# HarryShomer/LPFormer

Hardware: AMD Instinct MI355X
Metric: candidate link-pairs scored/sec (whole node) (higher is better)
Workload: dtype f32

## Files before the change

include/lpformer_hip.h:

```cpp
#ifndef LPFORMER_HIP_H
#define LPFORMER_HIP_H

#include <stdint.h>

#ifdef __cplusplus
extern "C" {
#endif

#define LPF_OK 0
#define LPF_ERR_INVALID (-1)
#define LPF_ERR_UNSUPPORTED (-2)
#define LPF_ERR_LAUNCH (-3)
#define LPF_ERR_NO_DEVICE (-4)

#define LPF_ABI_VERSION 10

#define LPF_FLAG_RELU 1u

int lpf_abi_version(void);
const char *lpf_strerror(int code);
const char *lpf_last_hip_error(void);
int lpf_device_info(int *cu_count, int *lds_bytes_per_cu, int *wave_size, char *arch_name, int arch_name_len);


int lpf_gcn_norm_csr(int64_t n, const int64_t *rowptr, const int32_t *col, const float *w_in,
                     float *w_out, float *dis_tmp, void *stream);

#define LPF_SPMM_LONG_ROW 128
int lpf_spmm_csr_f32(int64_t n, int32_t D, const int64_t *rowptr, const int32_t *col, const float *w,
                     const float *H, int64_t ldh, float *out, int64_t ldo, const float *bias,
// ... 215 lines not shown
                                 const float *pe_tab_signed, const float *pe_stat, const float *pat_base,
                                 const void *pat_grid, const void *pat_sign, int32_t grid_n, int32_t grid_shift,
                                 int32_t grid_base, float grid_ofs, const float *wfold_t, const float *att, const float *att_bias,
                                 const float *ln_g, const float *ln_b, int32_t n_counts, const int64_t *sel_ctl,
                                 float *pieces, int64_t units_cap, float *out, int64_t ldo, int32_t *perm,
                                 int64_t *n_nonempty, void *stream);
int lpf_pair_attention_rows4_zbf16(int32_t D, int64_t bs, const void *pair_tab, const int32_t *blk_cnt,
                                   const void *entries, int64_t ent_cap, const void *Z_bf16, int64_t ldz, const float *q,
                                   int64_t ldq, const float *pe_tab_signed, const float *pe_stat, const float *pat_base,
                                   const void *pat_grid, const void *pat_sign, int32_t grid_n, int32_t grid_shift,
                                   int32_t grid_base, float grid_ofs, const float *wfold_t, const float *att, const float *att_bias,
                                   const float *ln_g, const float *ln_b, int32_t n_counts, const int64_t *sel_ctl,
                                   float *pieces, int64_t units_cap, float *out, int64_t ldo, int32_t *perm,
                                   int64_t *n_nonempty, void *stream);

int lpf_tail_chain_rows_perm_f32(int64_t M, int32_t D, int32_t n_counts, const float *rows, int64_t ldrows,
                                 const float *wB_packed, const float *bB, const float *lnB_g, const float *lnB_b,
                                 const float *r_e, int64_t ldre, const float *wC_packed, const float *bC,
                                 const float *w_dot, const float *b_dot, const int64_t *sel_ctl, const int32_t *perm,
                                 const int64_t *n_full, const float *bC_empty, const float *row_empty, float *logit,
                                 float *prob, void *stream);
int lpf_tail_chain_rows_perm_bf16(int64_t M, int32_t D, int32_t n_counts, const float *rows, int64_t ldrows,
                                  const void *wB_packed_bf16, const float *bB, const float *lnB_g, const float *lnB_b,
                                  const float *r_e, int64_t ldre, const void *wC_packed_bf16, const float *bC,
                                  const float *w_dot, const float *b_dot, const int64_t *sel_ctl, const int32_t *perm,
                                  const int64_t *n_full, const float *bC_empty, const float *row_empty, float *logit,
                                  float *prob, void *stream);

int lpf_rowdot_sigmoid_f32(int64_t M, int32_t K, const float *A, int64_t lda, const float *w, float b,
                           float *logit, float *prob, void *stream);
// ... 64 lines not shown
```

lpformer_amd/_lib.py:

```python
from __future__ import annotations

import ctypes as C
import os
import threading

_HERE = os.path.dirname(os.path.abspath(__file__))
HIP_LIB_PATH = os.path.join(_HERE, "liblpformer_hip.so")
HOST_LIB_PATH = os.path.join(_HERE, "liblpformer_host.so")

ABI_VERSION = 10
FLAG_RELU = 1
SELECT_ERR_NODE_RANGE, SELECT_ERR_ITEM_CAP, SELECT_ERR_ENTRY_CAP = 1, 2, 4
ROWS_PERM_LB_WORDS = 1025
SELECT4_BLOCK = 64

i32, i64, f32, f64, u32, u64, vp = C.c_int32, C.c_int64, C.c_float, C.c_double, C.c_uint32, C.c_uint64, C.c_void_p

HIP_PROTOTYPES = {
    "lpf_abi_version": [],
    "lpf_strerror": [C.c_int],
    "lpf_last_hip_error": [],
    "lpf_device_info": [C.POINTER(C.c_int), C.POINTER(C.c_int), C.POINTER(C.c_int), C.c_char_p, C.c_int],
    "lpf_gcn_norm_csr": [i64, vp, vp, vp, vp, vp, vp],
    "lpf_spmm_csr_f32": [i64, i32, vp, vp, vp, vp, i64, vp, i64, vp, vp, vp, vp, i64, vp, vp, u32, vp, i64, vp],
    "lpf_gemm_f32": [i64, i32, i32, vp, i64, vp, i64, vp, vp, i64, vp, i64, u32, vp],
# ... 32 lines not shown
    "lpf_pair_attention_flip_f32": [i32, i64, vp, vp, i64, vp, i64, vp, i64, vp, vp, vp, vp, vp, vp, vp, i64, vp],
    "lpf_pair_attention_flip_zbf16": [i32, i64, vp, vp, i64, vp, i64, vp, i64, vp, vp, vp, vp, vp, vp, vp, i64, vp],
    "lpf_pair_attention_merge_f32": [i64, i32, i32, vp, vp, i64, vp, vp, vp, vp, vp, vp, i64, vp],
    "lpf_pair_attention_rows_f32": [i32, i64, vp, vp, i64, vp, i64, vp, i64, vp, vp, vp, vp, vp, vp, vp, vp, i32, vp, vp,
                                    i64, vp, i64, vp],
    "lpf_pair_attention_rows_zbf16": [i32, i64, vp, vp, i64, vp, i64, vp, i64, vp, vp, vp, vp, vp, vp, vp, vp, i32, vp, vp,
                                      i64, vp, i64, vp],
    "lpf_pair_attention_rows_perm_f32": [i32, i64, vp, vp, i64, vp, i64, vp, i64, vp, vp, vp, vp, vp, vp, vp, vp, i32, vp,
                                         vp, i64, vp, i64, vp, vp, vp, vp],
    "lpf_pair_attention_rows_perm_zbf16": [i32, i64, vp, vp, i64, vp, i64, vp, i64, vp, vp, vp, vp, vp, vp, vp, vp, i32,
                                           vp, vp, i64, vp, i64, vp, vp, vp, vp],
    "lpf_pair_attention_rows4_f32": [i32, i64, vp, vp, vp, i64, vp, i64, vp, i64, vp, vp, vp, vp, vp, i32, i32, i32, f32, vp,
                                     vp, vp, vp, vp, i32, vp, vp, i64, vp, i64, vp, vp, vp],
    "lpf_pair_attention_rows4_zbf16": [i32, i64, vp, vp, vp, i64, vp, i64, vp, i64, vp, vp, vp, vp, vp, i32, i32, i32, f32, vp,
                                       vp, vp, vp, vp, i32, vp, vp, i64, vp, i64, vp, vp, vp],
    "lpf_tail_chain_rows_perm_f32": [i64, i32, i32, vp, i64, vp, vp, vp, vp, vp, i64, vp, vp, vp, vp, vp, vp, vp, vp, vp,
                                     vp, vp, vp],
    "lpf_tail_chain_rows_perm_bf16": [i64, i32, i32, vp, i64, vp, vp, vp, vp, vp, i64, vp, vp, vp, vp, vp, vp, vp, vp, vp,
                                      vp, vp, vp],
    "lpf_pair_rows_piece_floats": [i32],
    "lpf_tail_chain_rows_f32": [i64, i32, i32, vp, i64, vp, vp, vp, vp, vp, i64, vp, vp, vp, vp, vp, vp, vp, vp],
    "lpf_tail_chain_rows_bf16": [i64, i32, i32, vp, i64, vp, vp, vp, vp, vp, i64, vp, vp, vp, vp, vp, vp, vp, vp],
    "lpf_tail_chain_merge_f32": [i64, i32, i32, vp, vp, i64, vp, vp, vp, vp, vp, vp, vp, vp, vp, i64, vp, vp, vp, vp, vp,
                                 vp, vp, vp],
    "lpf_tail_chain_merge_bf16": [i64, i32, i32, vp, vp, i64, vp, vp, vp, vp, vp, vp, vp, vp, vp, i64, vp, vp, vp, vp, vp,
                                 vp, vp, vp],
    "lpf_rowdot_sigmoid_f32": [i64, i32, vp, i64, vp, f32, vp, vp, vp],
    "lpf_tail_chain_f32": [i64, i32, i32, vp, i64, vp, vp, vp, vp, i64, vp, vp, vp, vp, vp, i64, vp, vp, vp, vp, vp,
                           vp, vp],
    "lpf_ppr_filter_count": [i64, vp, vp, i32, f32, vp, vp],
# ... 139 lines not shown
```

lpformer_amd/csrc/pair_rows.hip:

```cpp
#include <type_traits>

#include "pe_common.h"
#include "select_common.h"

namespace {

constexpr uint32_t PR_PAIR_MASK = 0x7fffffffu;
constexpr int PR_LB_WORDS = LPF_ROWS_PERM_LB_WORDS - 1;
#ifndef PR_CHUNK_N
#define PR_CHUNK_N 512
#endif
#ifndef PR_FLAGS_N
#define PR_FLAGS_N 2048
#endif
constexpr int PR_CHUNK = PR_CHUNK_N;
constexpr int PR_FLAGS = PR_FLAGS_N;

struct RowsArgs {
    int64_t bs;
    const int32_t *type_ptr;
    const int4 *entries;
    int64_t ent_cap;
    const float *Z; uint32_t ldz;
    const float *q; uint32_t ldq;
// ... 6 lines not shown
    float *out; int64_t ldo;
    int32_t n_counts;
    const int64_t *sel_ctl;
    float *pieces;
    int64_t units_cap;
    int32_t *perm;
    uint64_t *perm_lb;
    int64_t *n_nonempty;
    const int4 *pair_tab;
    const int32_t *blk_cnt;
    const float *pat_base;
    const uint8_t *pat_grid;
    const uint32_t *pat_sign;
    int32_t grid_n, grid_shift, grid_base;
    float grid_ofs;
};

template <int CTRL>
__device__ __forceinline__ float pr_dpp(float v) {
    return __builtin_bit_cast(float, __builtin_amdgcn_update_dpp(0, __builtin_bit_cast(int, v), CTRL, 0xf, 0xf, false));
}
template <int G>
__device__ __forceinline__ float pr_group_sum(float v) {
    v += pr_dpp<0xB1>(v);
    v += pr_dpp<0x4E>(v);
    if constexpr (G >= 8) v += pr_dpp<0x141>(v);
    if constexpr (G >= 16) v += pr_dpp<0x140>(v);
    if constexpr (G >= 32)
        v += __builtin_bit_cast(float, __builtin_amdgcn_ds_swizzle(__builtin_bit_cast(int, v), 0x401f));
    if constexpr (G >= 64) {
// ... 32 lines not shown
    static constexpr int WT = STAT + 6;
    static constexpr int REC = WT + (PT ? 0 : WTL) * D * GG;
    static constexpr int SC = REC + NG * 16;
    static constexpr int META = SC + NG * 8;
    static constexpr int TP = META + NG * 4;
    static constexpr int CUM = TP + 3 * (PR_CHUNK / 4 + 1);
    static constexpr int LISTS = CUM + (PR_CHUNK / 4 + 1);
    static constexpr int CTL = LISTS + 2 * (PR_CHUNK / 4);
    static constexpr int FLAGS = CTL + 4;
    static constexpr int WCNT = FLAGS + PR_FLAGS / 4;
    static constexpr int SIGN = WCNT + 8;
    static constexpr int TOTAL = SIGN + (PT ? (3 * NP * ((D + 31) / 32) + 3) / 4 : 0);
    static constexpr size_t BYTES = (size_t)TOTAL * 16;
};

template <int G, int NTH, int WTL_, bool ZB = false, bool PT = false, int NV = 1>
__global__ __launch_bounds__(NTH, NTH >= 512 ? 4 : 3) void pair_rows_kernel(const RowsArgs A) {
    using ZT = typename std::conditional<ZB, uint2, float4>::type;
    using L = PrLds<G, NTH, WTL_, PT, NV>;
    constexpr int WTL = PT ? 0 : WTL_, NP = L::NP, GG = L::GG;
    constexpr int D = 4 * GG, EPW = 64 / G, NG = L::NG, T_LO = WTL == 1 ? 1 : 0, TPS = PR_CHUNK + 4, RSP = pr_piece_floats(D);
    constexpr uint32_t PAIR_MASK = PT ? 0x1fffffffu : PR_PAIR_MASK;
    constexpr int SB = LPF_SELECT4_BLOCK;
    constexpr int EW = 4;
    extern __shared__ __attribute__((aligned(16))) float4 pr_lds[];
    float4 *const ltab = pr_lds + L::TAB;
    float4 *const lbase = pr_lds + L::BASE;
    float4 *const lvec = pr_lds + L::VEC;
    float4 *const lconst = pr_lds + L::CONST_ROW;
    float *const lstat = reinterpret_cast<float *>(pr_lds + L::STAT);
    float4 *const lwt = pr_lds + L::WT;
    int4 *const lrec = reinterpret_cast<int4 *>(pr_lds + L::REC);
    f32x2 *const lsc = reinterpret_cast<f32x2 *>(pr_lds + L::SC);
    int *const lmeta = reinterpret_cast<int *>(pr_lds + L::META);
    int *const ltp = reinterpret_cast<int *>(pr_lds + L::TP);
    int *const lcum = reinterpret_cast<int *>(pr_lds + L::CUM);
    int *const llist = reinterpret_cast<int *>(pr_lds + L::LISTS);
    int *const lctl = reinterpret_cast<int *>(pr_lds + L::CTL);
// ... 361 lines not shown
        if constexpr (ZB)
            return make_float4(__uint_as_float(z.x << 16), __uint_as_float(z.x & 0xffff0000u),
                               __uint_as_float(z.y << 16), __uint_as_float(z.y & 0xffff0000u));
        else
            return z;
    };
    auto grid_cell = [&](float v) __attribute__((always_inline)) {
        const int c = (int)(__float_as_uint(v + A.grid_ofs) >> A.grid_shift) - A.grid_base;
        return c < 0 ? A.grid_n - 1 : (c < A.grid_n ? c : A.grid_n - 1);
    };
    auto q_row = [&](int pair, float4 (&q)[NV]) __attribute__((always_inline)) {
#pragma unroll
        for (int v = 0; v < NV; ++v)
            q[v] = *reinterpret_cast<const float4 *>(A.q + (uint64_t)(uint32_t)pair * A.ldq + off + 4 * G * v);
    };

    for (int64_t c0 = P0; c0 < P1; c0 += PR_CHUNK) {
        const int cn = (int)(P1 - c0 < PR_CHUNK ? P1 - c0 : PR_CHUNK);
        constexpr int PER = (PR_CHUNK + NTH - 1) / NTH;
        int4 e_pre[PER];
        if constexpr (PT) {
#pragma unroll
            for (int i = 0; i < PER; ++i) {
                const int k = tid * PER + i;
                e_pre[i] = A.pair_tab[c0 + (k < cn ? k : cn - 1)];
            }
        }
        pr_lds_barrier();
        int64_t v0, v1;
        if constexpr (PT) {
// ... 55 lines not shown
        const int64_t u_first = v0 >> 4;
        const int n_units = v1 > v0 ? (int)(((v1 - 1) >> 4) - u_first + 1) : 0;
        const bool inl = n_units <= PR_FLAGS;
        if (inl)
            for (int k = tid; k < n_units; k += NTH) lflag[k] = 0;
        pr_lds_barrier();
        PR_STAMP(2);
        PR_STAMP(3);
        while (true) {
            int tk = 0;
            if (lane == 0) tk = atomicAdd(&lctl[2], 1);
            tk = __builtin_amdgcn_readfirstlane(tk);
            if (tk * EPW >= n_units) break;
            const int ul = tk * EPW + grp;
            const int64_t x0 = (u_first + ul) << 4;
            for (int i = lj; i < 16; i += G) {
                int4 rec = make_int4(0, 0, 0, 0);
                int meta = 0;
                f32x2 sc = {0.f, 0.f};
                const int64_t x = x0 + i;
                if (ul < n_units && x >= v0 && x < v1) {
                    const int xr = (int)(x - v0);
                    int lo = 0, hi = cn;
                    while (hi - lo > 1) {
                        const int mid = (lo + hi) >> 1;
                        if (lcum[mid] <= xr) lo = mid; else hi = mid;
                    }
                    const int k = lo, ps = lcum[k], pe = lcum[k + 1], j = xr - ps;
                    int t;
                    if constexpr (PT) {
                        rec = A.entries[(int64_t)ltp[k] + j];
                        t = (int)(((uint32_t)rec.x >> 29) & 3u) - 1;
                        t = t < 0 ? 0 : t;
                    } else {
                        const int *tp = ltp + k;
                        const int lo0 = tp[0], n0 = tp[1] - lo0, lo1 = tp[TPS], n1 = tp[TPS + 1] - lo1, lo2 = tp[2 * TPS];
                        t = (j >= n0) + (j >= n0 + n1);
                        const int64_t idx = t == 0 ? lo0 + j : (t == 1 ? lo1 + (j - n0) : lo2 + (j - n0 - n1));
                        rec = A.entries[(int64_t)t * A.ent_cap + idx];
                    }
                    const int64_t ustart = x0 - v0, uend = ustart + 16;
                    const bool head = ps < ustart, more = pe > uend;
                    meta = t | ((j == 0 || i == 0) ? 4 : 0) | ((xr == pe - 1 || i == 15) ? 8 : 0) |
                           ((head || more) ? 16 : 0) | (head ? 32 : 0) | 64 | ((head && !more && inl) ? 128 : 0);
                    const float *st = lstat + 8 * t;
                    const float pa = __int_as_float(rec.z), pb = __int_as_float(rec.w);
// ... 14 lines not shown
                    }
                    const float vab = st[0] * pa * pa + st[1] * pb * pb + st[2] + 2.0f * (st[3] * pa * pb + st[4] * pa + st[5] * pb);
                    const float vba = st[0] * pb * pb + st[1] * pa * pa + st[2] + 2.0f * (st[3] * pa * pb + st[4] * pb + st[5] * pa);
                    sc = f32x2{__builtin_amdgcn_rsqf(fmaxf(vab, 0.0f) + 1e-5f), __builtin_amdgcn_rsqf(fmaxf(vba, 0.0f) + 1e-5f)};
                }
                lr[i] = rec;
                lm[i] = meta;
                ls[i] = sc;
            }
            int lro = 0;
            asm volatile("s_waitcnt vmcnt(0) lgkmcnt(0)" : "+v"(lro) :: "memory");
            constexpr int ZBATCH = NV == 1 ? 4 : 1;
            ZT za[ZBATCH][NV], zb[ZBATCH][NV];
#pragma unroll
            for (int u = 0; u < ZBATCH; ++u) z_row(lr[lro + u].y, za[u]);
            float4 qc[NV];
            q_row((int)((uint32_t)lr[lro].x & PAIR_MASK), qc);
            float *const piece_u = A.pieces + (u_first + ul) * 2 * RSP;
            float m = -INFINITY, l = 0.f;
            Q4 o[NV];
            q4_zero(o);
            int hpair = -1;

            auto entry = [&](const int i, const ZT (&zraw)[NV]) __attribute__((always_inline)) {
                const int4 rc = lr[lro + i];
                const f32x2 r12 = ls[lro + i];
                const int meta = lm[lro + i];
                const int pair_n = (int)((uint32_t)lr[lro + (i < 15 ? i + 1 : 15)].x & PAIR_MASK);
                const int pair_i = (int)((uint32_t)rc.x & PAIR_MASK);
                const bool on = meta & 64;
                const int t = meta & 3;
                const float pa = __int_as_float(rc.z), pb = __int_as_float(rc.w);
                const f32x2 pab = {pa, pb}, pba = {pb, pa};
                const float4 *tabl = ltab + t * GG + lj;
                Q4 k[NV];
                if constexpr (PT) {
                    const int i1 = (meta >> 9) & 63, i2 = (meta >> 15) & 63;
                    const float4 *b1 = lbase + i1 * D + lj, *b2 = lbase + i2 * D + lj;
                    const f32x2 c1 = r12.x * pab, c2 = r12.y * pba;
#pragma unroll
                    for (int v = 0; v < NV; ++v) {
                        const float4 zc = z_wide(zraw[v]);
                        const float4 P1 = b1[v * G], Q1 = b1[GG + v * G], R1 = b1[2 * GG + v * G], B1 = b1[3 * GG + v * G];
                        k[v].a = f32x2{zc.x, zc.y} + (f32x2{P1.x, P1.y} * c1.x + (f32x2{Q1.x, Q1.y} * c1.y +
                                                      (f32x2{R1.x, R1.y} * r12.x + f32x2{B1.x, B1.y})));
                        k[v].b = f32x2{zc.z, zc.w} + (f32x2{P1.z, P1.w} * c1.x + (f32x2{Q1.z, Q1.w} * c1.y +
                                                      (f32x2{R1.z, R1.w} * r12.x + f32x2{B1.z, B1.w})));
                    }
#pragma unroll
                    for (int v = 0; v < NV; ++v) {
                        const float4 P2 = b2[v * G], Q2 = b2[GG + v * G], R2 = b2[2 * GG + v * G], B2 = b2[3 * GG + v * G];
                        k[v].a += f32x2{P2.x, P2.y} * c2.x + (f32x2{Q2.x, Q2.y} * c2.y + (f32x2{R2.x, R2.y} * r12.y + f32x2{B2.x, B2.y}));
                        k[v].b += f32x2{P2.z, P2.w} * c2.x + (f32x2{Q2.z, Q2.w} * c2.y + (f32x2{R2.z, R2.w} * r12.y + f32x2{B2.z, B2.w}));
                    }
                } else {
                    const float4 *basel = lbase + t * D + lj;
                    const f32x2 cab = r12.x * pab + r12.y * pba;
                    const float cr = r12.x + r12.y;
#pragma unroll
                    for (int v = 0; v < NV; ++v) {
                        const float4 zc = z_wide(zraw[v]);
                        const float4 P0v = basel[v * G], Q0v = basel[GG + v * G], R0v = basel[2 * GG + v * G], C0v = basel[3 * GG + v * G];
                        k[v].a = f32x2{zc.x, zc.y} + (f32x2{P0v.x, P0v.y} * cab.x +
                                                      (f32x2{Q0v.x, Q0v.y} * cab.y + (f32x2{R0v.x, R0v.y} * cr + f32x2{C0v.x, C0v.y})));
                        k[v].b = f32x2{zc.z, zc.w} + (f32x2{P0v.z, P0v.w} * cab.x +
                                                      (f32x2{Q0v.z, Q0v.w} * cab.y + (f32x2{R0v.z, R0v.w} * cr + f32x2{C0v.z, C0v.w})));
                    }
                }
// ... 65 lines not shown
                                }
                                vp = mine ? val : 0.f;
                            }
                        }
#pragma unroll
                        for (int v = 0; v < NV; ++v) {
                            k[v].a += wp[v].a * vp;
                            k[v].b += wp[v].b * vp;
                        }
                    }
                }
                }
                f32x2 sp = {0.f, 0.f};
#pragma unroll
                for (int v = 0; v < NV; ++v) {
                    const f32x2 x01 = k[v].a * f32x2{qc[v].x, qc[v].y}, x23 = k[v].b * f32x2{qc[v].z, qc[v].w};
                    const f32x2 y01 = x01 * 0.2f, y23 = x23 * 0.2f;
                    const f32x2 l01 = {fmaxf(x01.x, y01.x), fmaxf(x01.y, y01.y)}, l23 = {fmaxf(x23.x, y23.x), fmaxf(x23.y, y23.y)};
                    if (v == 0) sp = l01 * at01[v] + l23 * at23[v];
                    else sp += l01 * at01[v] + l23 * at23[v];
                }
                const float s = pr_group_sum<G>(sp.x + sp.y);
                if (on) {
                    if (meta & 4) {
                        m = -INFINITY; l = 0.f;
                        q4_zero(o);
                    }
                    const float d = s - m;
                    const float e = __expf(-fabsf(d));
                    const bool up = d > 0.f;
                    const float sca = up ? e : 1.f, w = up ? 1.f : e;
// ... 7 lines not shown
                    if (meta & 8) {
                        if (meta & 128) hpair = pair_i;
                        if (meta & 16) {
                            float *dst = piece_u + ((meta & 32) ? 0 : RSP);
#pragma unroll
                            for (int v = 0; v < NV; ++v)
                                *reinterpret_cast<float4 *>(dst + off + 4 * G * v) = make_float4(o[v].a.x, o[v].a.y, o[v].b.x, o[v].b.y);
                            if (lj == 0) *reinterpret_cast<float2 *>(dst + D) = make_float2(m, l);
                        } else {
                            float4 r[NV];
                            finish_row(o, l, r);
                            store_row(pair_i, r);
                        }
                    }
                }
                if (pair_n != pair_i) q_row(pair_n, qc);
                __builtin_amdgcn_sched_barrier(0);
            };
            auto batch = [&](const int qt, const ZT (&zc4)[ZBATCH][NV], ZT (&zn4)[ZBATCH][NV]) __attribute__((always_inline)) {
                constexpr int NQ = 16 / ZBATCH;
                const int nb = qt < NQ - 1 ? ZBATCH * qt + ZBATCH : 16 - ZBATCH;
#pragma unroll
                for (int u = 0; u < ZBATCH; ++u) z_row(lr[lro + nb + u].y, zn4[u]);
                __builtin_amdgcn_sched_barrier(0);
#pragma unroll
                for (int u = 0; u < ZBATCH; ++u) entry(ZBATCH * qt + u, zc4[u]);
            };
#pragma unroll 1
            for (int h = 0; h < 8 / ZBATCH; ++h) {
                batch(2 * h, za, zb);
                batch(2 * h + 1, zb, za);
// ... 174 lines not shown
            pr_lds_barrier();
            ne_base += tot_ne;
        }
    }
#ifdef PR_STAMPS
    if (lane == 0 && pr_stamp_buf) {
        uint64_t *o = pr_stamp_buf + ((int64_t)blockIdx.x * (NTH / 64) + wave) * 8;
        for (int k = 0; k < 6; ++k) o[k] = st_t[k];
        o[3] = st_t[7];
        o[6] = (uint64_t)st_rounds;
        o[7] = (uint64_t)(P1 - P0) | ((uint64_t)lctl[1] << 32);
    }
#endif
}

template <bool ZB, bool PT = false>
int rows_launch(int32_t D, int64_t bs, const int32_t *type_ptr, const void *entries, int64_t ent_cap, const void *Z,
                int64_t ldz, const float *q, int64_t ldq, const float *pe_tab_signed, const float *pe_stat,
                const float *base, const float *wfold_t, const float *att, const float *att_bias, const float *ln_g,
                const float *ln_b, int32_t n_counts, const int64_t *sel_ctl, float *pieces, int64_t units_cap, float *out,
                int64_t ldo, void *stream, int32_t *perm = nullptr, uint64_t *perm_lb = nullptr,
                int64_t *n_nonempty = nullptr, const void *pair_tab = nullptr, const int32_t *blk_cnt = nullptr,
                const float *pat_base = nullptr, const uint8_t *pat_grid = nullptr, const uint32_t *pat_sign = nullptr,
                int32_t grid_n = 0,
                int32_t grid_shift = 0, int32_t grid_base = 0, float grid_ofs = 0.f) {
    if (bs == 0) return LPF_OK;
    LPF_REQUIRE(!PT || (pat_base && pat_grid && pat_sign && lpf_aligned16(pat_base) && grid_n >= 2 && grid_n <= 4096 &&
                        grid_shift >= 0 && grid_shift <= 23 && grid_base >= 0 && grid_ofs >= 0.f));
    LPF_REQUIRE(bs > 0 && bs < (PT ? (1ll << 29) : (1ll << 31)) &&
                (PT ? (pair_tab && blk_cnt && lpf_aligned16(pair_tab) && (reinterpret_cast<uintptr_t>(blk_cnt) & 7) == 0)
                    : type_ptr != nullptr) &&
                entries && ent_cap > 0 && ent_cap < (PT ? (1ll << 31) : (1ll << 29)) && Z && q &&
                pe_tab_signed && pe_stat && (PT || base) && wfold_t && att && att_bias && ln_g && ln_b && out && pieces &&
                units_cap >= (PT ? 2 : (3 * ent_cap + 15) / 16 + 1) && lpf_aligned16(pieces));
    LPF_REQUIRE(!perm || ((PT || perm_lb) && n_nonempty));
    LPF_REQUIRE((n_counts == 0 || n_counts == 1 || n_counts == 3 || n_counts == 4) && ldo >= D + n_counts && (ldo & 3) == 0);
    LPF_REQUIRE(ldz >= D && ldq >= D && ldz < (1ll << 31) && ldq < (1ll << 31) && (ldz & (ZB ? 7 : 3)) == 0 &&
                (ldq & 3) == 0 && lpf_aligned16(entries) && lpf_aligned16(Z) && lpf_aligned16(q) &&
                lpf_aligned16(pe_tab_signed) && (PT || lpf_aligned16(base)) && lpf_aligned16(wfold_t) && lpf_aligned16(att) &&
                lpf_aligned16(att_bias) && lpf_aligned16(ln_g) && lpf_aligned16(ln_b) && lpf_aligned16(out));
    const RowsArgs a{bs, type_ptr, static_cast<const int4 *>(entries), ent_cap, static_cast<const float *>(Z), (uint32_t)ldz,
                     q, (uint32_t)ldq, pe_tab_signed, pe_stat, base, wfold_t, att, att_bias, ln_g, ln_b, out, ldo,
                     n_counts, sel_ctl, pieces, units_cap, perm, perm_lb, n_nonempty,
                     static_cast<const int4 *>(pair_tab), blk_cnt, pat_base, pat_grid, pat_sign, grid_n, grid_shift, grid_base,
                     grid_ofs};
    hipStream_t s = static_cast<hipStream_t>(stream);
    const int n_cu = lpf_cu_count();
    if (n_cu == 0) return LPF_ERR_NO_DEVICE;
#ifdef PR_GRID2
#define PR_GRID_MUL 2
#else
#define PR_GRID_MUL 1
#endif
#define LPF_ROWS_GO(GQ, NTH, WTL, PER_CU, NVV)                                                      \
    do {                                                                                            \
        auto kern = pair_rows_kernel<GQ, NTH, WTL, ZB, PT, NVV>;                                        \
        constexpr size_t lds = PrLds<GQ, NTH, WTL, PT, NVV>::BYTES;                                 \
        LPF_SET_MAX_LDS(kern, lds);                                                                 \
        int64_t groups = (int64_t)n_cu * PER_CU * PR_GRID_MUL;                                      \
        const int64_t most = (bs + 15) / 16;      \
        if (groups > most) groups = most;                                                           \
        if (groups > PR_LB_WORDS) groups = PR_LB_WORDS;                                             \
        hipLaunchKernelGGL(kern, dim3((unsigned)groups), dim3(NTH), lds, s, a);                     \
    } while (0)
    switch (D) {
        case 32: LPF_ROWS_GO(8, 512, 3, 2, 1); break;
        case 64: LPF_ROWS_GO(16, 512, 3, 2, 1); break;
#ifdef PR_CFG128
#define LPF_ROWS_GO_(...) LPF_ROWS_GO(__VA_ARGS__)
        case 128: LPF_ROWS_GO_(PR_CFG128); break;
#undef LPF_ROWS_GO_
#else
        case 128:
            if constexpr (PT) LPF_ROWS_GO(16, 1024, 0, 1, 2);
            else LPF_ROWS_GO(32, 1024, 1, 1, 1);
            break;
#endif
        case 256:
            if constexpr (PT) LPF_ROWS_GO(32, 1024, 0, 1, 2);
            else LPF_ROWS_GO(64, 256, 0, 3, 1);
            break;
        default: return LPF_ERR_UNSUPPORTED;
// ... 81 lines not shown
                                              const float *q, int64_t ldq, const float *pe_tab_signed,
                                              const float *pe_stat, const float *pat_base, const void *pat_grid,
                                              const void *pat_sign, int32_t grid_n, int32_t grid_shift, int32_t grid_base,
                                              float grid_ofs,
                                              const float *wfold_t, const float *att, const float *att_bias,
                                              const float *ln_g, const float *ln_b, int32_t n_counts,
                                              const int64_t *sel_ctl, float *pieces, int64_t units_cap, float *out,
                                              int64_t ldo, int32_t *perm, int64_t *n_nonempty, void *stream) {
    return rows_launch<true, true>(D, bs, nullptr, entries, ent_cap, Z_bf16, ldz, q, ldq, pe_tab_signed, pe_stat, nullptr,
                                   wfold_t, att, att_bias, ln_g, ln_b, n_counts, sel_ctl, pieces, units_cap, out, ldo, stream,
                                   perm, nullptr, n_nonempty, pair_tab, blk_cnt, pat_base,
                                   static_cast<const uint8_t *>(pat_grid), static_cast<const uint32_t *>(pat_sign), grid_n,
                                   grid_shift, grid_base, grid_ofs);
}

extern "C" int64_t lpf_pair_rows_piece_floats(int32_t D) { return pr_piece_floats(D); }
```

lpformer_amd/link_transformer.py:

```python
from __future__ import annotations

import functools
import math
import weakref
from typing import Optional

import numpy as np
import torch
import torch.nn as nn

from . import _lib, fold, graph, mask_delta, patterns
from . import dist as lpf_dist
from ._lib import FLAG_RELU, check, ptr
from .profile import KernelTimer


def _stream(device):
    idx = device.index if isinstance(device, torch.device) and device.index is not None else torch.cuda.current_device()
    return torch._C._cuda_getCurrentRawStream(idx)


def _on_device(fn):
    @functools.wraps(fn)
    def wrapper(self, *args, **kwargs):
# ... 1429 lines not shown
            self._fold()
            last = getattr(self, "_auto_choice", None)
            if last is not None and (last[0] is self._folded[0] or self.training or
                                     self._refolds - last[2] < self.flip_recheck_every):
                return last[1]
            if self.training:
                return "flip"
            choice = "flip" if self.flips_per_entry() <= self.flip_break_even() else "mfma"
            self._auto_choice = (self._folded[0], choice, self._refolds)
            return choice
        return self.attention_impl

    def _uses_rows(self) -> bool:
        return self.attention_rows and self.attention_kernel() == "flip"

    def _attention_rows(self, batch, x_node, test_set, adj_mask, side, out, n_counts, order=False, q=None):
        lib, st, d = _lib.hip(), _stream(self.device), self.dim
        bs = batch.shape[1]
        w = self._fold()
        z = self._node_keys(x_node, w)
        if q is None:
            with torch.cuda.stream(side if side is not None else torch.cuda.current_stream(self.device)):
                q = self._pair_q(batch, x_node, w)
        four = self._uses_select4(adj_mask)
        ws = self._select4_device(batch, test_set) if four else self._select_device(batch, test_set, adj_mask)
        if side is not None:
            _lib.stream_wait(torch.cuda.current_stream(self.device), side)
        layer = self.att_layers[0]
        units_cap = (ws.kept_cap + 15) // 16 + 1 if four else (3 * ws.ent_cap + 15) // 16 + 1
        pieces = self._workspace("att_pieces", units_cap * 2 * int(lib.lpf_pair_rows_piece_floats(d)), torch.float32, st)
        extra = ()
        if order:
            perm = self._workspace("att_perm", bs, torch.int32, st)
            nfull = self._workspace("att_nfull", 1, torch.int64, st)
            extra = (ptr(perm), ptr(nfull)) if four else \
                (ptr(perm), ptr(self._zero_workspace("att_perm_lb", 2 * _lib.ROWS_PERM_LB_WORDS, st)), ptr(nfull))
        zt = self._z_bf16(z) if self.precision == "bf16" else z
        if four:
            pt = self._pattern_tables(w)
            geo = pt["geo"]
            bases = (ptr(pt["base"]), ptr(pt["grid"]), ptr(pt["sign"]), geo["n"], geo["shift"], geo["base"], geo["ofs"])
        else:
            bases = (ptr(w["flip_base"]),)
        tabs = (ptr(zt), zt.stride(0), ptr(q), q.stride(0), ptr(w["flip_tab"]), ptr(w["pe_stat"]), *bases,
                ptr(w["wfold_t"]), ptr(w["att"]), ptr(layer.att.bias), ptr(layer.post_att_norm.weight),
                ptr(layer.post_att_norm.bias), n_counts, ptr(ws.ctl), ptr(pieces), units_cap, ptr(out), out.stride(0))
        with KernelTimer.span("pair_attention_rows"):
            if four:
                name = "lpf_pair_attention_rows4" + ("_zbf16" if self.precision == "bf16" else "_f32")
                check(getattr(lib, name)(d, bs, ptr(ws.pair_tab), ptr(ws.blk_cnt), ptr(ws.entries), ws.ent_cap, *tabs,
                                         *(extra or (None, None)), st), name)
            else:
                name = ("lpf_pair_attention_rows" + ("_perm" if order else "") +
                        ("_zbf16" if self.precision == "bf16" else "_f32"))
                check(getattr(lib, name)(d, bs, ptr(ws.type_ptr), ptr(ws.entries), ws.ent_cap, *tabs, *extra, st), name)
        return (ws, perm, nfull) if order else ws

    def _fused_attention(self, batch, x_node, test_set, adj_mask, side, q=None):
        lib, st, d = _lib.hip(), _stream(self.device), self.dim
        bs = batch.shape[1]
        w = self._fold()
        z = self._node_keys(x_node, w)
        if q is None:
            with torch.cuda.stream(side if side is not None else torch.cuda.current_stream(self.device)):
# ... 175 lines not shown
            return self._score_pairs_folded(batch, X_node, score_func, test_set, adj_mask, logits)
        finally:
            self._fold_memo = None

    def _score_pairs_folded(self, batch, X_node, score_func, test_set, adj_mask, logits):
        with torch.no_grad():
            d, pd = self.dim, self.dim + self.count_dim
            batch = self._prep_batch(batch)
            bs = batch.shape[1]
            x_node = _as_f32_rows(X_node)
            a, c, kpad = self._score_fold(score_func)
            r = torch.empty(bs, kpad, dtype=torch.float32, device=self.device)
            ew, pw = self.elementwise_lin, self.pairwise_lin
            one_pass = d in (32, 64, 128, 256) and self.use_tail_chain and self.use_fused_attention and bs > 0
            q_side = None
            if one_pass and self.query_from == "table" and (d < 256 or self._uses_rows()):
                q_side = (self._node_y(x_node, self._fold()), torch.empty(bs, d, dtype=torch.float32, device=self.device))
            if one_pass:
                self._prepare_pair_major(adj_mask)
            side = self._fork()
            with torch.cuda.stream(side if side is not None else torch.cuda.current_stream(self.device)):
                t = ew._chain1.tables(ew.linears[0].weight, ew.linears[0].bias, ew.norm.weight, ew.norm.bias)
                if ew._chain1.run(t, x_node, relu=True, batch=batch, in_mode=1, out=r[:, :d], side=q_side) is None:
                    q_side = None
                    prod = torch.empty(bs, d, dtype=torch.float32, device=self.device)
                    with KernelTimer.span("pair_gather"):
                        check(_lib.hip().lpf_pair_gather_f32(bs, d, ptr(batch), batch.stride(0), x_node.shape[0], ptr(x_node),
                                                             x_node.stride(0), ptr(prod), d, None, 0,
                                                             _stream(self.device)), "lpf_pair_gather_f32")
                    gemm(prod, ew._pads[0].get(ew.linears[0].weight), ew.linears[0].bias, out=r[:, :d])
                    layernorm_(r[:, :d], ew.norm.weight, ew.norm.bias, relu=True)
            if (d in (32, 64, 128, 256) and self.use_tail_chain and self.use_fused_attention and bs > 0 and
                    (self._uses_rows() or d == 256)):
                lib, st = _lib.hip(), _stream(self.device)
# ... 131 lines not shown
```

Before: 251.6 million.

## Compute pair query from node Y table inside rows4 attention kernel

Adds a YQ variant of the rows4 pair-attention kernel that reads the two endpoint rows of the per-node Y table via the batch indices and sums them in-kernel, instead of materialising a per-pair q buffer through a separate pass. The Python path selects this variant for dim>=128, table queries, f32 precision and select4. It also adds a wave-uniform fast path that reuses the same LDS basis loads when both count indices match across the wave. In exchange there are two Y row loads per pair change and extra batch-index loads and shuffles in the staging loop.

After: 240.3 million (median of 2 runs). -4.5%, worse.

```diff
diff --git a/include/lpformer_hip.h b/include/lpformer_hip.h
--- a/include/lpformer_hip.h
+++ b/include/lpformer_hip.h
@@ -13,7 +13,7 @@
 #define LPF_ERR_LAUNCH (-3)
 #define LPF_ERR_NO_DEVICE (-4)
 
-#define LPF_ABI_VERSION 10
+#define LPF_ABI_VERSION 11
 
 #define LPF_FLAG_RELU 1u
 
@@ -259,6 +259,25 @@
                                    float *pieces, int64_t units_cap, float *out, int64_t ldo, int32_t *perm,
                                    int64_t *n_nonempty, void *stream);
 
+int lpf_pair_attention_rows4_yq_f32(int32_t D, int64_t bs, const void *pair_tab, const int32_t *blk_cnt, const void *entries,
+                                    int64_t ent_cap, const float *Z, int64_t ldz, const float *Y, int64_t ldy,
+                                    int64_t n_rows, const int64_t *batch, int64_t batch_ld, const float *pe_tab_signed,
+                                    const float *pe_stat, const float *pat_base, const void *pat_grid, const void *pat_sign,
+                                    int32_t grid_n, int32_t grid_shift, int32_t grid_base, float grid_ofs,
+                                    const float *wfold_t, const float *att, const float *att_bias, const float *ln_g,
+                                    const float *ln_b, int32_t n_counts, const int64_t *sel_ctl, float *pieces,
+                                    int64_t units_cap, float *out, int64_t ldo, int32_t *perm, int64_t *n_nonempty,
+                                    void *stream);
+int lpf_pair_attention_rows4_yq_zbf16(int32_t D, int64_t bs, const void *pair_tab, const int32_t *blk_cnt,
+                                      const void *entries, int64_t ent_cap, const void *Z_bf16, int64_t ldz, const float *Y,
+                                      int64_t ldy, int64_t n_rows, const int64_t *batch, int64_t batch_ld,
+                                      const float *pe_tab_signed, const float *pe_stat, const float *pat_base,
+                                      const void *pat_grid, const void *pat_sign, int32_t grid_n, int32_t grid_shift,
+                                      int32_t grid_base, float grid_ofs, const float *wfold_t, const float *att,
+                                      const float *att_bias, const float *ln_g, const float *ln_b, int32_t n_counts,
+                                      const int64_t *sel_ctl, float *pieces, int64_t units_cap, float *out, int64_t ldo,
+                                      int32_t *perm, int64_t *n_nonempty, void *stream);
+
 int lpf_tail_chain_rows_perm_f32(int64_t M, int32_t D, int32_t n_counts, const float *rows, int64_t ldrows,
                                  const float *wB_packed, const float *bB, const float *lnB_g, const float *lnB_b,
                                  const float *r_e, int64_t ldre, const float *wC_packed, const float *bC,
diff --git a/lpformer_amd/_lib.py b/lpformer_amd/_lib.py
--- a/lpformer_amd/_lib.py
+++ b/lpformer_amd/_lib.py
@@ -8,7 +8,7 @@
 HIP_LIB_PATH = os.path.join(_HERE, "liblpformer_hip.so")
 HOST_LIB_PATH = os.path.join(_HERE, "liblpformer_host.so")
 
-ABI_VERSION = 10
+ABI_VERSION = 11
 FLAG_RELU = 1
 SELECT_ERR_NODE_RANGE, SELECT_ERR_ITEM_CAP, SELECT_ERR_ENTRY_CAP = 1, 2, 4
 ROWS_PERM_LB_WORDS = 1025
@@ -71,6 +71,10 @@
                                      vp, vp, vp, vp, i32, vp, vp, i64, vp, i64, vp, vp, vp],
     "lpf_pair_attention_rows4_zbf16": [i32, i64, vp, vp, vp, i64, vp, i64, vp, i64, vp, vp, vp, vp, vp, i32, i32, i32, f32, vp,
                                        vp, vp, vp, vp, i32, vp, vp, i64, vp, i64, vp, vp, vp],
+    "lpf_pair_attention_rows4_yq_f32": [i32, i64, vp, vp, vp, i64, vp, i64, vp, i64, i64, vp, i64, vp, vp, vp, vp, vp, i32,
+                                        i32, i32, f32, vp, vp, vp, vp, vp, i32, vp, vp, i64, vp, i64, vp, vp, vp],
+    "lpf_pair_attention_rows4_yq_zbf16": [i32, i64, vp, vp, vp, i64, vp, i64, vp, i64, i64, vp, i64, vp, vp, vp, vp, vp, i32,
+                                          i32, i32, f32, vp, vp, vp, vp, vp, i32, vp, vp, i64, vp, i64, vp, vp, vp],
     "lpf_tail_chain_rows_perm_f32": [i64, i32, i32, vp, i64, vp, vp, vp, vp, vp, i64, vp, vp, vp, vp, vp, vp, vp, vp, vp,
                                      vp, vp, vp],
     "lpf_tail_chain_rows_perm_bf16": [i64, i32, i32, vp, i64, vp, vp, vp, vp, vp, i64, vp, vp, vp, vp, vp, vp, vp, vp, vp,
diff --git a/lpformer_amd/csrc/pair_rows.hip b/lpformer_amd/csrc/pair_rows.hip
--- a/lpformer_amd/csrc/pair_rows.hip
+++ b/lpformer_amd/csrc/pair_rows.hip
@@ -44,6 +44,8 @@
     const uint32_t *pat_sign;
     int32_t grid_n, grid_shift, grid_base;
     float grid_ofs;
+    const float *Y; uint32_t ldy;
+    const int64_t *batch; int64_t batch_ld, n_rows;
 };
 
 template <int CTRL>
@@ -106,7 +108,7 @@
     static constexpr size_t BYTES = (size_t)TOTAL * 16;
 };
 
-template <int G, int NTH, int WTL_, bool ZB = false, bool PT = false, int NV = 1>
+template <int G, int NTH, int WTL_, bool ZB = false, bool PT = false, int NV = 1, bool YQ = false>
 __global__ __launch_bounds__(NTH, NTH >= 512 ? 4 : 3) void pair_rows_kernel(const RowsArgs A) {
     using ZT = typename std::conditional<ZB, uint2, float4>::type;
     using L = PrLds<G, NTH, WTL_, PT, NV>;
@@ -114,6 +116,7 @@
     constexpr int D = 4 * GG, EPW = 64 / G, NG = L::NG, T_LO = WTL == 1 ? 1 : 0, TPS = PR_CHUNK + 4, RSP = pr_piece_floats(D);
     constexpr uint32_t PAIR_MASK = PT ? 0x1fffffffu : PR_PAIR_MASK;
     constexpr int SB = LPF_SELECT4_BLOCK;
+    static_assert(!YQ || (PT && G >= 16), "the query from Y: PT form, one staging lane per entry");
     constexpr int EW = 4;
     extern __shared__ __attribute__((aligned(16))) float4 pr_lds[];
     float4 *const ltab = pr_lds + L::TAB;
@@ -505,6 +508,13 @@
         for (int v = 0; v < NV; ++v)
             q[v] = *reinterpret_cast<const float4 *>(A.q + (uint64_t)(uint32_t)pair * A.ldq + off + 4 * G * v);
     };
+    auto y_rows = [&](int ya, int yb, float4 (&qa)[NV], float4 (&qb)[NV]) __attribute__((always_inline)) {
+#pragma unroll
+        for (int v = 0; v < NV; ++v) {
+            qa[v] = *reinterpret_cast<const float4 *>(A.Y + (uint64_t)(uint32_t)ya * A.ldy + off + 4 * G * v);
+            qb[v] = *reinterpret_cast<const float4 *>(A.Y + (uint64_t)(uint32_t)yb * A.ldy + off + 4 * G * v);
+        }
+    };
 
     for (int64_t c0 = P0; c0 < P1; c0 += PR_CHUNK) {
         const int cn = (int)(P1 - c0 < PR_CHUNK ? P1 - c0 : PR_CHUNK);
@@ -590,6 +600,7 @@
             if (tk * EPW >= n_units) break;
             const int ul = tk * EPW + grp;
             const int64_t x0 = (u_first + ul) << 4;
+            int id_a = 0, id_b = 0;
             for (int i = lj; i < 16; i += G) {
                 int4 rec = make_int4(0, 0, 0, 0);
                 int meta = 0;
@@ -606,6 +617,11 @@
                     int t;
                     if constexpr (PT) {
                         rec = A.entries[(int64_t)ltp[k] + j];
+                        if constexpr (YQ) {
+                            const int64_t ia = A.batch[c0 + k], ib = A.batch[A.batch_ld + c0 + k];
+                            id_a = (uint64_t)ia < (uint64_t)A.n_rows ? (int)ia : 0;
+                            id_b = (uint64_t)ib < (uint64_t)A.n_rows ? (int)ib : 0;
+                        }
                         t = (int)(((uint32_t)rec.x >> 29) & 3u) - 1;
                         t = t < 0 ? 0 : t;
                     } else {
@@ -650,8 +666,15 @@
             ZT za[ZBATCH][NV], zb[ZBATCH][NV];
 #pragma unroll
             for (int u = 0; u < ZBATCH; ++u) z_row(lr[lro + u].y, za[u]);
-            float4 qc[NV];
-            q_row((int)((uint32_t)lr[lro].x & PAIR_MASK), qc);
+            float4 qc[NV], qb[NV];
+#ifdef PR_YQ_NOW
+            if constexpr (YQ) { y_rows(__shfl(id_a, grp * G, 64), __shfl(id_b, grp * G, 64), qc, qb);
+#pragma unroll
+                for (int v = 0; v < NV; ++v) qc[v] = make_float4(qc[v].x + qb[v].x, qc[v].y + qb[v].y, qc[v].z + qb[v].z, qc[v].w + qb[v].w); }
+#else
+            if constexpr (YQ) y_rows(__shfl(id_a, grp * G, 64), __shfl(id_b, grp * G, 64), qc, qb);
+#endif
+            else q_row((int)((uint32_t)lr[lro].x & PAIR_MASK), qc);
             float *const piece_u = A.pieces + (u_first + ul) * 2 * RSP;
             float m = -INFINITY, l = 0.f;
             Q4 o[NV];
@@ -674,20 +697,36 @@
                     const int i1 = (meta >> 9) & 63, i2 = (meta >> 15) & 63;
                     const float4 *b1 = lbase + i1 * D + lj, *b2 = lbase + i2 * D + lj;
                     const f32x2 c1 = r12.x * pab, c2 = r12.y * pba;
-#pragma unroll
-                    for (int v = 0; v < NV; ++v) {
-                        const float4 zc = z_wide(zraw[v]);
-                        const float4 P1 = b1[v * G], Q1 = b1[GG + v * G], R1 = b1[2 * GG + v * G], B1 = b1[3 * GG + v * G];
-                        k[v].a = f32x2{zc.x, zc.y} + (f32x2{P1.x, P1.y} * c1.x + (f32x2{Q1.x, Q1.y} * c1.y +
-                                                      (f32x2{R1.x, R1.y} * r12.x + f32x2{B1.x, B1.y})));
-                        k[v].b = f32x2{zc.z, zc.w} + (f32x2{P1.z, P1.w} * c1.x + (f32x2{Q1.z, Q1.w} * c1.y +
-                                                      (f32x2{R1.z, R1.w} * r12.x + f32x2{B1.z, B1.w})));
-                    }
-#pragma unroll
-                    for (int v = 0; v < NV; ++v) {
-                        const float4 P2 = b2[v * G], Q2 = b2[GG + v * G], R2 = b2[2 * GG + v * G], B2 = b2[3 * GG + v * G];
-                        k[v].a += f32x2{P2.x, P2.y} * c2.x + (f32x2{Q2.x, Q2.y} * c2.y + (f32x2{R2.x, R2.y} * r12.y + f32x2{B2.x, B2.y}));
-                        k[v].b += f32x2{P2.z, P2.w} * c2.x + (f32x2{Q2.z, Q2.w} * c2.y + (f32x2{R2.z, R2.w} * r12.y + f32x2{B2.z, B2.w}));
+                    auto first = [&](const float4 &zc, const float4 &P1, const float4 &Q1, const float4 &R1, const float4 &B1,
+                                     Q4 &kv) __attribute__((always_inline)) {
+                        kv.a = f32x2{zc.x, zc.y} + (f32x2{P1.x, P1.y} * c1.x + (f32x2{Q1.x, Q1.y} * c1.y +
+                                                    (f32x2{R1.x, R1.y} * r12.x + f32x2{B1.x, B1.y})));
+                        kv.b = f32x2{zc.z, zc.w} + (f32x2{P1.z, P1.w} * c1.x + (f32x2{Q1.z, Q1.w} * c1.y +
+                                                    (f32x2{R1.z, R1.w} * r12.x + f32x2{B1.z, B1.w})));
+                    };
+                    auto second = [&](const float4 &P2, const float4 &Q2, const float4 &R2, const float4 &B2, Q4 &kv)
+                        __attribute__((always_inline)) {
+                        kv.a += f32x2{P2.x, P2.y} * c2.x + (f32x2{Q2.x, Q2.y} * c2.y + (f32x2{R2.x, R2.y} * r12.y + f32x2{B2.x, B2.y}));
+                        kv.b += f32x2{P2.z, P2.w} * c2.x + (f32x2{Q2.z, Q2.w} * c2.y + (f32x2{R2.z, R2.w} * r12.y + f32x2{B2.z, B2.w}));
+                    };
+#ifdef PR_NO_REUSE
+                    if (false) {
+#else
+                    if (!__ballot(i1 != i2)) {
+#endif
+#pragma unroll
+                        for (int v = 0; v < NV; ++v) {
+                            const float4 P1 = b1[v * G], Q1 = b1[GG + v * G], R1 = b1[2 * GG + v * G], B1 = b1[3 * GG + v * G];
+                            first(z_wide(zraw[v]), P1, Q1, R1, B1, k[v]);
+                            second(P1, Q1, R1, B1, k[v]);
+                        }
+                    } else {
+#pragma unroll
+                        for (int v = 0; v < NV; ++v)
+                            first(z_wide(zraw[v]), b1[v * G], b1[GG + v * G], b1[2 * GG + v * G], b1[3 * GG + v * G], k[v]);
+#pragma unroll
+                        for (int v = 0; v < NV; ++v)
+                            second(b2[v * G], b2[GG + v * G], b2[2 * GG + v * G], b2[3 * GG + v * G], k[v]);
                     }
                 } else {
                     const float4 *basel = lbase + t * D + lj;
@@ -783,7 +822,11 @@
                 f32x2 sp = {0.f, 0.f};
 #pragma unroll
                 for (int v = 0; v < NV; ++v) {
-                    const f32x2 x01 = k[v].a * f32x2{qc[v].x, qc[v].y}, x23 = k[v].b * f32x2{qc[v].z, qc[v].w};
+                    float4 qv = qc[v];
+#ifndef PR_YQ_NOW
+                    if constexpr (YQ) qv = make_float4(qc[v].x + qb[v].x, qc[v].y + qb[v].y, qc[v].z + qb[v].z, qc[v].w + qb[v].w);
+#endif
+                    const f32x2 x01 = k[v].a * f32x2{qv.x, qv.y}, x23 = k[v].b * f32x2{qv.z, qv.w};
                     const f32x2 y01 = x01 * 0.2f, y23 = x23 * 0.2f;
                     const f32x2 l01 = {fmaxf(x01.x, y01.x), fmaxf(x01.y, y01.y)}, l23 = {fmaxf(x23.x, y23.x), fmaxf(x23.y, y23.y)};
                     if (v == 0) sp = l01 * at01[v] + l23 * at23[v];
@@ -821,7 +864,21 @@
                         }
                     }
                 }
-                if (pair_n != pair_i) q_row(pair_n, qc);
+                if constexpr (YQ) {
+                    if (__ballot(pair_n != pair_i)) {
+                        const int src = grp * G + (i < 15 ? i + 1 : 15);
+                        const int na = __shfl(id_a, src, 64), nb = __shfl(id_b, src, 64);
+                        if (pair_n != pair_i) {
+                            y_rows(na, nb, qc, qb);
+#ifdef PR_YQ_NOW
+#pragma unroll
+                            for (int v = 0; v < NV; ++v) qc[v] = make_float4(qc[v].x + qb[v].x, qc[v].y + qb[v].y, qc[v].z + qb[v].z, qc[v].w + qb[v].w);
+#endif
+                        }
+                    }
+                } else if (pair_n != pair_i) {
+                    q_row(pair_n, qc);
+                }
                 __builtin_amdgcn_sched_barrier(0);
             };
             auto batch = [&](const int qt, const ZT (&zc4)[ZBATCH][NV], ZT (&zn4)[ZBATCH][NV]) __attribute__((always_inline)) {
@@ -1026,7 +1083,7 @@
 #endif
 }
 
-template <bool ZB, bool PT = false>
+template <bool ZB, bool PT = false, bool YQ = false>
 int rows_launch(int32_t D, int64_t bs, const int32_t *type_ptr, const void *entries, int64_t ent_cap, const void *Z,
                 int64_t ldz, const float *q, int64_t ldq, const float *pe_tab_signed, const float *pe_stat,
                 const float *base, const float *wfold_t, const float *att, const float *att_bias, const float *ln_g,
@@ -1035,8 +1092,12 @@
                 int64_t *n_nonempty = nullptr, const void *pair_tab = nullptr, const int32_t *blk_cnt = nullptr,
                 const float *pat_base = nullptr, const uint8_t *pat_grid = nullptr, const uint32_t *pat_sign = nullptr,
                 int32_t grid_n = 0,
-                int32_t grid_shift = 0, int32_t grid_base = 0, float grid_ofs = 0.f) {
+                int32_t grid_shift = 0, int32_t grid_base = 0, float grid_ofs = 0.f, const float *Y = nullptr,
+                int64_t ldy = 0, int64_t n_rows = 0, const int64_t *batch = nullptr, int64_t batch_ld = 0) {
     if (bs == 0) return LPF_OK;
+    LPF_REQUIRE(!YQ || (Y && batch && n_rows > 0 && ldy >= D && ldy < (1ll << 31) && (ldy & 3) == 0 && lpf_aligned16(Y) &&
+                        batch_ld >= bs && (D == 128 || D == 256)));
+    if constexpr (YQ) { q = Y; ldq = ldy; }
     LPF_REQUIRE(!PT || (pat_base && pat_grid && pat_sign && lpf_aligned16(pat_base) && grid_n >= 2 && grid_n <= 4096 &&
                         grid_shift >= 0 && grid_shift <= 23 && grid_base >= 0 && grid_ofs >= 0.f));
     LPF_REQUIRE(bs > 0 && bs < (PT ? (1ll << 29) : (1ll << 31)) &&
@@ -1055,7 +1116,7 @@
                      q, (uint32_t)ldq, pe_tab_signed, pe_stat, base, wfold_t, att, att_bias, ln_g, ln_b, out, ldo,
                      n_counts, sel_ctl, pieces, units_cap, perm, perm_lb, n_nonempty,
                      static_cast<const int4 *>(pair_tab), blk_cnt, pat_base, pat_grid, pat_sign, grid_n, grid_shift, grid_base,
-                     grid_ofs};
+                     grid_ofs, Y, (uint32_t)ldy, batch, batch_ld, n_rows};
     hipStream_t s = static_cast<hipStream_t>(stream);
     const int n_cu = lpf_cu_count();
     if (n_cu == 0) return LPF_ERR_NO_DEVICE;
@@ -1066,7 +1127,7 @@
 #endif
 #define LPF_ROWS_GO(GQ, NTH, WTL, PER_CU, NVV)                                                      \
     do {                                                                                            \
-        auto kern = pair_rows_kernel<GQ, NTH, WTL, ZB, PT, NVV>;                                        \
+        auto kern = pair_rows_kernel<GQ, NTH, WTL, ZB, PT, NVV, YQ>;                                    \
         constexpr size_t lds = PrLds<GQ, NTH, WTL, PT, NVV>::BYTES;                                 \
         LPF_SET_MAX_LDS(kern, lds);                                                                 \
         int64_t groups = (int64_t)n_cu * PER_CU * PR_GRID_MUL;                                      \
@@ -1076,8 +1137,8 @@
         hipLaunchKernelGGL(kern, dim3((unsigned)groups), dim3(NTH), lds, s, a);                     \
     } while (0)
     switch (D) {
-        case 32: LPF_ROWS_GO(8, 512, 3, 2, 1); break;
-        case 64: LPF_ROWS_GO(16, 512, 3, 2, 1); break;
+        case 32: if constexpr (!YQ) LPF_ROWS_GO(8, 512, 3, 2, 1); break;
+        case 64: if constexpr (!YQ) LPF_ROWS_GO(16, 512, 3, 2, 1); break;
 #ifdef PR_CFG128
 #define LPF_ROWS_GO_(...) LPF_ROWS_GO(__VA_ARGS__)
         case 128: LPF_ROWS_GO_(PR_CFG128); break;
@@ -1189,4 +1250,38 @@
                                    grid_shift, grid_base, grid_ofs);
 }
 
+extern "C" int lpf_pair_attention_rows4_yq_f32(int32_t D, int64_t bs, const void *pair_tab, const int32_t *blk_cnt,
+                                               const void *entries, int64_t ent_cap, const float *Z, int64_t ldz,
+                                               const float *Y, int64_t ldy, int64_t n_rows, const int64_t *batch,
+                                               int64_t batch_ld, const float *pe_tab_signed, const float *pe_stat,
+                                               const float *pat_base, const void *pat_grid, const void *pat_sign,
+                                               int32_t grid_n, int32_t grid_shift, int32_t grid_base, float grid_ofs,
+                                               const float *wfold_t, const float *att, const float *att_bias,
+                                               const float *ln_g, const float *ln_b, int32_t n_counts,
+                                               const int64_t *sel_ctl, float *pieces, int64_t units_cap, float *out,
+                                               int64_t ldo, int32_t *perm, int64_t *n_nonempty, void *stream) {
+    return rows_launch<false, true, true>(D, bs, nullptr, entries, ent_cap, Z, ldz, nullptr, 0, pe_tab_signed, pe_stat,
+                                          nullptr, wfold_t, att, att_bias, ln_g, ln_b, n_counts, sel_ctl, pieces, units_cap,
+                                          out, ldo, stream, perm, nullptr, n_nonempty, pair_tab, blk_cnt, pat_base,
+                                          static_cast<const uint8_t *>(pat_grid), static_cast<const uint32_t *>(pat_sign),
+                                          grid_n, grid_shift, grid_base, grid_ofs, Y, ldy, n_rows, batch, batch_ld);
+}
+
+extern "C" int lpf_pair_attention_rows4_yq_zbf16(int32_t D, int64_t bs, const void *pair_tab, const int32_t *blk_cnt,
+                                                 const void *entries, int64_t ent_cap, const void *Z_bf16, int64_t ldz,
+                                                 const float *Y, int64_t ldy, int64_t n_rows, const int64_t *batch,
+                                                 int64_t batch_ld, const float *pe_tab_signed, const float *pe_stat,
+                                                 const float *pat_base, const void *pat_grid, const void *pat_sign,
+                                                 int32_t grid_n, int32_t grid_shift, int32_t grid_base, float grid_ofs,
+                                                 const float *wfold_t, const float *att, const float *att_bias,
+                                                 const float *ln_g, const float *ln_b, int32_t n_counts,
+                                                 const int64_t *sel_ctl, float *pieces, int64_t units_cap, float *out,
+                                                 int64_t ldo, int32_t *perm, int64_t *n_nonempty, void *stream) {
+    return rows_launch<true, true, true>(D, bs, nullptr, entries, ent_cap, Z_bf16, ldz, nullptr, 0, pe_tab_signed, pe_stat,
+                                         nullptr, wfold_t, att, att_bias, ln_g, ln_b, n_counts, sel_ctl, pieces, units_cap,
+                                         out, ldo, stream, perm, nullptr, n_nonempty, pair_tab, blk_cnt, pat_base,
+                                         static_cast<const uint8_t *>(pat_grid), static_cast<const uint32_t *>(pat_sign),
+                                         grid_n, grid_shift, grid_base, grid_ofs, Y, ldy, n_rows, batch, batch_ld);
+}
+
 extern "C" int64_t lpf_pair_rows_piece_floats(int32_t D) { return pr_piece_floats(D); }
diff --git a/lpformer_amd/link_transformer.py b/lpformer_amd/link_transformer.py
--- a/lpformer_amd/link_transformer.py
+++ b/lpformer_amd/link_transformer.py
@@ -1467,12 +1467,17 @@
     def _uses_rows(self) -> bool:
         return self.attention_rows and self.attention_kernel() == "flip"
 
+    def _rows_yq(self, adj_mask=None) -> bool:
+        return (self.dim >= 128 and self.query_from == "table" and self.precision != "bf16" and self._uses_rows() and
+                self._uses_select4(adj_mask))
+
     def _attention_rows(self, batch, x_node, test_set, adj_mask, side, out, n_counts, order=False, q=None):
         lib, st, d = _lib.hip(), _stream(self.device), self.dim
         bs = batch.shape[1]
         w = self._fold()
         z = self._node_keys(x_node, w)
-        if q is None:
+        y = self._node_y(x_node, w) if q is None and self._rows_yq(adj_mask) else None
+        if q is None and y is None:
             with torch.cuda.stream(side if side is not None else torch.cuda.current_stream(self.device)):
                 q = self._pair_q(batch, x_node, w)
         four = self._uses_select4(adj_mask)
@@ -1495,12 +1500,14 @@
             bases = (ptr(pt["base"]), ptr(pt["grid"]), ptr(pt["sign"]), geo["n"], geo["shift"], geo["base"], geo["ofs"])
         else:
             bases = (ptr(w["flip_base"]),)
-        tabs = (ptr(zt), zt.stride(0), ptr(q), q.stride(0), ptr(w["flip_tab"]), ptr(w["pe_stat"]), *bases,
+        qtab = (ptr(y), y.stride(0), y.shape[0], ptr(batch), batch.stride(0)) if y is not None else (ptr(q), q.stride(0))
+        tabs = (ptr(zt), zt.stride(0), *qtab, ptr(w["flip_tab"]), ptr(w["pe_stat"]), *bases,
                 ptr(w["wfold_t"]), ptr(w["att"]), ptr(layer.att.bias), ptr(layer.post_att_norm.weight),
                 ptr(layer.post_att_norm.bias), n_counts, ptr(ws.ctl), ptr(pieces), units_cap, ptr(out), out.stride(0))
         with KernelTimer.span("pair_attention_rows"):
             if four:
-                name = "lpf_pair_attention_rows4" + ("_zbf16" if self.precision == "bf16" else "_f32")
+                name = ("lpf_pair_attention_rows4" + ("_yq" if y is not None else "") +
+                        ("_zbf16" if self.precision == "bf16" else "_f32"))
                 check(getattr(lib, name)(d, bs, ptr(ws.pair_tab), ptr(ws.blk_cnt), ptr(ws.entries), ws.ent_cap, *tabs,
                                          *(extra or (None, None)), st), name)
             else:
@@ -1706,10 +1713,12 @@
             ew, pw = self.elementwise_lin, self.pairwise_lin
             one_pass = d in (32, 64, 128, 256) and self.use_tail_chain and self.use_fused_attention and bs > 0
             q_side = None
-            if one_pass and self.query_from == "table" and (d < 256 or self._uses_rows()):
+            if one_pass and self.query_from == "table" and (d < 256 or self._uses_rows()) and not self._rows_yq(adj_mask):
                 q_side = (self._node_y(x_node, self._fold()), torch.empty(bs, d, dtype=torch.float32, device=self.device))
             if one_pass:
                 self._prepare_pair_major(adj_mask)
+                if self._rows_yq(adj_mask):
+                    self._node_y(x_node, self._fold())
             side = self._fork()
             with torch.cuda.stream(side if side is not None else torch.cuda.current_stream(self.device)):
                 t = ew._chain1.tables(ew.linears[0].weight, ew.linears[0].bias, ew.norm.weight, ew.norm.bias)
```
